# bruAristimunha/Synthetic-Sleep-EEG-Signal-Generation-using-Latent-Diffusion-Models

Measured on AMD Instinct MI355X. Metric: EEG windows/sec (LDM train step), higher is better.
Workload: dtype bf16; 1 GPU; LDM train step on raw (B,1,3072) windows: frozen AutoencoderKL[32,32,64] encode+sample x scale, add_noise, config_ldm.yaml UNet (30.5M params, latent_channels=1) fwd+bwd, epsilon MSE, Adam lr 1e-4 [BASELINE configs[2]/[3]: per-GPU batch 256 = global 2048 / 8]; per_gpu_batch=256, global_batch=256, latent_len=768, parallelism=dp1

## Files before the change

### synthetic-sleep-eeg-signal-generation-using-latent-diffusion-models_amd/csrc/conv_ws.hip

```cpp
#include <stdlib.h>

#include "common.h"
#include "internal.h"

namespace {
constexpr int WS_ROWS = 64;
constexpr int WS_BUF_ROWS = 68;
constexpr int WS_ROW_BYTES = 256;
constexpr int WS_ABUF = WS_BUF_ROWS * WS_ROW_BYTES;
constexpr int WS_OUT = WS_ROWS * WS_ROW_BYTES;
constexpr int WS_RING = 3;
constexpr int WS_LDS = WS_RING * WS_ABUF + WS_OUT;

struct WsArgs {
  const bf16_t* x; long ldx;
  const bf16_t* w; long sWt, sWn, sWk; int tflip;
  const float* bias; const float* rowvec; long ld_rowvec;
  const bf16_t* resid; long ldr;
  bf16_t* y; long ldy;
  int M, L, N, ntiles, tiles_per_block;
  const void* zero_page;
  float* col_parts;
};

typedef unsigned u32x2 __attribute__((ext_vector_type(2)));

__device__ __forceinline__ void ws_barrier() {
  asm volatile("s_waitcnt lgkmcnt(0)" ::: "memory");
  __builtin_amdgcn_s_barrier();
  asm volatile("" ::: "memory");
}

__device__ __forceinline__ void ws_dma16(const void* g, unsigned lds_off) {
  asm volatile("s_mov_b32 m0, %0\n\ts_nop 0\n\tglobal_load_lds_dwordx4 %1, off" ::"s"(lds_off), "v"(g) : "memory", "m0");
}
__device__ __forceinline__ u32x2 ws_load8(const void* g) {
  u32x2 r;
  asm volatile("global_load_dwordx2 %0, %1, off" : "=v"(r) : "v"(g) : "memory");
  return r;
}

__device__ __forceinline__ float ws_row16_sum(float v) {
  v += __builtin_bit_cast(float, __builtin_amdgcn_update_dpp(0, __builtin_bit_cast(int, v), 0xB1, 0xF, 0xF, true));
  v += __builtin_bit_cast(float, __builtin_amdgcn_update_dpp(0, __builtin_bit_cast(int, v), 0x4E, 0xF, 0xF, true));
  v += __builtin_bit_cast(float, __builtin_amdgcn_update_dpp(0, __builtin_bit_cast(int, v), 0x141, 0xF, 0xF, true));
  v += __builtin_bit_cast(float, __builtin_amdgcn_update_dpp(0, __builtin_bit_cast(int, v), 0x140, 0xF, 0xF, true));
  return v;
}
__device__ __forceinline__ void ws_col_stats(float (&cs)[2][4], float (&cq)[2][4], float* __restrict__ row, int n0, int lm, int q) {
#pragma unroll
  for (int cf = 0; cf < 2; cf++)
#pragma unroll
    for (int r = 0; r < 4; r++) {
      const float a = ws_row16_sum(cs[cf][r]), b = ws_row16_sum(cq[cf][r]);
      if (lm == 0) *(float2*)(row + 2 * (n0 + cf * 16 + q * 4 + r)) = make_float2(a, b);
    }
}

template <bool TR, typename T16 = bf16_t, bool ST = false>
__global__ __launch_bounds__(256, 2) void conv3_ws_kernel(const WsArgs p) {
  extern __shared__ __attribute__((aligned(1024))) char smem[];
  const int tid = threadIdx.x, wave = tid >> 6, lane = tid & 63, lm = lane & 15, q = lane >> 4;
  const int n0 = blockIdx.y * 128 + wave * 32;
  const int t_begin = blockIdx.x * p.tiles_per_block;
  int t_end = t_begin + p.tiles_per_block; if (t_end > p.ntiles) t_end = p.ntiles;
  if (t_begin >= t_end) return;
  const unsigned lds_base = (unsigned)(size_t)(__attribute__((address_space(3))) char*)smem;
  const int wave_u = __builtin_amdgcn_readfirstlane(wave);

  auto issue_dma = [&](int t) {
    const int buf = (t - t_begin) % WS_RING;
    const long row0 = (long)t * WS_ROWS;
    const bool has_left = (row0 % p.L) != 0, has_right = ((row0 + WS_ROWS) % p.L) != 0;
    for (int i = wave_u; i < WS_BUF_ROWS / 4; i += 4) {
      const int j = 4 * i + q, c = lm ^ (j & 15);
      const bool ok = (j >= 1 && j <= WS_ROWS) || (j == 0 && has_left) || (j == WS_ROWS + 1 && has_right);
      const char* src = ok ? (const char*)(p.x + (row0 - 1 + j) * p.ldx) + c * 16 : (const char*)p.zero_page;
      ws_dma16(src, __builtin_amdgcn_readfirstlane(lds_base + buf * WS_ABUF + i * 1024));
    }
  };
  issue_dma(t_begin);
  if (t_begin + 1 < t_end) issue_dma(t_begin + 1);

  uint4 wf[3][4][2];
#pragma unroll
  for (int t = 0; t < 3; t++) {
    const bf16_t* wt = p.w + (long)(p.tflip ? 2 - t : t) * p.sWt;
#pragma unroll
    for (int kk = 0; kk < 4; kk++)
#pragma unroll
      for (int cf = 0; cf < 2; cf++) {
        const bf16_t* wp = wt + (long)(n0 + cf * 16 + lm) * p.sWn + (long)(kk * 32 + q * 8) * p.sWk;
        if constexpr (!TR) wf[t][kk][cf] = *(const uint4*)wp;
        else {
          unsigned e[8];
#pragma unroll
          for (int i = 0; i < 8; i++) e[i] = wp[(long)i * p.sWk];
          wf[t][kk][cf] = make_uint4(e[0] | (e[1] << 16), e[2] | (e[3] << 16), e[4] | (e[5] << 16), e[6] | (e[7] << 16));
        }
      }
  }
  float4 bv[2], ev[2];
#pragma unroll
  for (int cf = 0; cf < 2; cf++) bv[cf] = p.bias ? *(const float4*)(p.bias + n0 + cf * 16 + q * 4) : make_float4(0.f, 0.f, 0.f, 0.f);
  int ev_sample = -1;
  __builtin_amdgcn_s_waitcnt(0x0F70);

  char* sOut = smem + WS_RING * WS_ABUF;
  auto store_tile = [&](int t) {
    const long row0 = (long)t * WS_ROWS;
#pragma unroll
    for (int i = 0; i < 4; i++) {
      const int c = tid + 256 * i, row = c >> 4, ch = c & 15;
      const uint4 v = *(const uint4*)(sOut + row * WS_ROW_BYTES + ((ch ^ (row & 15)) * 16));
      *(uint4*)(p.y + (row0 + row) * p.ldy + blockIdx.y * 128 + ch * 8) = v;
    }
  };

  float cs[2][4], cq[2][4];
#pragma unroll
  for (int cf = 0; cf < 2; cf++)
#pragma unroll
    for (int r = 0; r < 4; r++) { cs[cf][r] = 0.f; cq[cf][r] = 0.f; }
  for (int t = t_begin; t < t_end; t++) {
    const int buf = (t - t_begin) % WS_RING;
    const long row0 = (long)t * WS_ROWS;
    if (t + 1 < t_end) asm volatile("s_waitcnt vmcnt(4)" ::: "memory"); else asm volatile("s_waitcnt vmcnt(0)" ::: "memory");
    ws_barrier();
    if (t > t_begin) store_tile(t - 1);
    const int sample = (int)(row0 / p.L);
    if (sample != ev_sample) {
      ev_sample = sample;
#pragma unroll
      for (int cf = 0; cf < 2; cf++) {
        ev[cf] = bv[cf];
        if (p.rowvec) {
          const float4 e = *(const float4*)(p.rowvec + (long)sample * p.ld_rowvec + n0 + cf * 16 + q * 4);
          ev[cf].x += e.x; ev[cf].y += e.y; ev[cf].z += e.z; ev[cf].w += e.w;
        }
      }
    }
    u32x2 rr[4][2];
    if (p.resid) {
#pragma unroll
      for (int rf = 0; rf < 4; rf++)
#pragma unroll
        for (int cf = 0; cf < 2; cf++) rr[rf][cf] = ws_load8(p.resid + (row0 + rf * 16 + lm) * p.ldr + n0 + cf * 16 + q * 4);
    }
    const bool more = t + 2 < t_end;
    if (more) issue_dma(t + 2);

    const char* sA = smem + buf * WS_ABUF;
    f32x4 acc[4][2];
#pragma unroll
    for (int rf = 0; rf < 4; rf++)
#pragma unroll
      for (int cf = 0; cf < 2; cf++) acc[rf][cf] = (f32x4){0.f, 0.f, 0.f, 0.f};
#pragma unroll
    for (int rf = 0; rf < 4; rf++)
#pragma unroll
      for (int tp = 0; tp < 3; tp++) {
        const int j = rf * 16 + lm + tp;
#pragma unroll
        for (int kk = 0; kk < 4; kk++) {
          const uint4 xf = *(const uint4*)(sA + j * WS_ROW_BYTES + (((kk * 4 + q) ^ (j & 15)) * 16));
#pragma unroll
          for (int cf = 0; cf < 2; cf++)
            if constexpr (Is16<T16>::f16) acc[rf][cf] = __builtin_amdgcn_mfma_f32_16x16x32_f16(__builtin_bit_cast(f16x8, wf[tp][kk][cf]), __builtin_bit_cast(f16x8, xf), acc[rf][cf], 0, 0, 0);
            else acc[rf][cf] = __builtin_amdgcn_mfma_f32_16x16x32_bf16(__builtin_bit_cast(bf16x8, wf[tp][kk][cf]), __builtin_bit_cast(bf16x8, xf), acc[rf][cf], 0, 0, 0);
        }
      }
    if (p.resid) {
      if (!more) asm volatile("s_waitcnt vmcnt(0)" ::: "memory");
      asm volatile("s_waitcnt vmcnt(4)" : "+v"(rr[0][0]), "+v"(rr[0][1]), "+v"(rr[1][0]), "+v"(rr[1][1]), "+v"(rr[2][0]), "+v"(rr[2][1]), "+v"(rr[3][0]), "+v"(rr[3][1]) :: "memory");
    }
    ws_barrier();
#pragma unroll
    for (int rf = 0; rf < 4; rf++)
#pragma unroll
      for (int cf = 0; cf < 2; cf++) {
        float v0 = acc[rf][cf][0] + ev[cf].x, v1 = acc[rf][cf][1] + ev[cf].y, v2 = acc[rf][cf][2] + ev[cf].z, v3 = acc[rf][cf][3] + ev[cf].w;
        if (p.resid) {
          v0 += w16_lo<T16>(rr[rf][cf].x); v1 += w16_hi<T16>(rr[rf][cf].x);
          v2 += w16_lo<T16>(rr[rf][cf].y); v3 += w16_hi<T16>(rr[rf][cf].y);
        }
        if constexpr (ST) {
          cs[cf][0] += v0; cs[cf][1] += v1; cs[cf][2] += v2; cs[cf][3] += v3;
          cq[cf][0] = fmaf(v0, v0, cq[cf][0]); cq[cf][1] = fmaf(v1, v1, cq[cf][1]); cq[cf][2] = fmaf(v2, v2, cq[cf][2]); cq[cf][3] = fmaf(v3, v3, cq[cf][3]);
        }
        const int row = rf * 16 + lm, ch = wave * 4 + cf * 2 + (q >> 1);
        *(uint2*)(sOut + row * WS_ROW_BYTES + ((ch ^ (row & 15)) * 16) + (q & 1) * 8) = make_uint2(pack16x2<T16>(v0, v1), pack16x2<T16>(v2, v3));
      }
  }
  ws_barrier();
  store_tile(t_end - 1);
  if constexpr (ST) ws_col_stats(cs, cq, p.col_parts + (size_t)blockIdx.x * 2 * p.N, n0, lm, q);
}

constexpr int W2_ROWS = 32, W2_BUF_ROWS = 36, W2_ROW_BYTES = 512;
constexpr int W2_ABUF = W2_BUF_ROWS * W2_ROW_BYTES;
constexpr int W2_OUT = W2_ROWS * 256;
constexpr int W2_LDS = WS_RING * W2_ABUF + W2_OUT;

struct Ws2Args {
  const bf16_t* x; long ldx;
  const bf16_t* w;
  const float* bias;
  bf16_t* y; long ldy;
  int M, L, ntiles, tiles_per_block;
  const void* zero_page;
  float* col_parts;
};

template <int MODE> struct W2Map;
template <> struct W2Map<0> { static constexpr int SLOTS = 12; static __device__ __forceinline__ void at(int s, int& tp, int& kk) { if (s < 4) { tp = 0; kk = 4 + s; } else { tp = 1; kk = s - 4; } } };
template <> struct W2Map<1> { static constexpr int SLOTS = 8;  static __device__ __forceinline__ void at(int s, int& tp, int& kk) { tp = 1; kk = s; } };
template <> struct W2Map<2> { static constexpr int SLOTS = 16; static __device__ __forceinline__ void at(int s, int& tp, int& kk) { tp = 1 + (s >> 3); kk = s & 7; } };

template <int MODE, typename T16, bool ST = false>
__device__ __forceinline__ void ws2_body(const Ws2Args& p, char* smem) {
  using Map = W2Map<MODE>;
  const int tid = threadIdx.x, wave = tid >> 6, lane = tid & 63, lm = lane & 15, q = lane >> 4;
  const int nb0 = blockIdx.y * 128, n0 = nb0 + wave * 32;
  const int t_begin = blockIdx.x * p.tiles_per_block;
  int t_end = t_begin + p.tiles_per_block; if (t_end > p.ntiles) t_end = p.ntiles;
  if (t_begin >= t_end) return;
  const unsigned lds_base = (unsigned)(size_t)(__attribute__((address_space(3))) char*)smem;
  const int wave_u = __builtin_amdgcn_readfirstlane(wave);
  auto issue_dma = [&](int t) {
    const int buf = (t - t_begin) % WS_RING;
    const long row0 = (long)t * W2_ROWS;
    const bool has_left = (row0 % p.L) != 0, has_right = ((row0 + W2_ROWS) % p.L) != 0;
    for (int i = wave_u; i < W2_BUF_ROWS / 2; i += 4) {
      const int j = 2 * i + (lane >> 5), c = (lane & 31) ^ (j & 15);
      const bool ok = (j >= 1 && j <= W2_ROWS) || (j == 0 && has_left) || (j == W2_ROWS + 1 && has_right);
      const char* src = ok ? (const char*)(p.x + (row0 - 1 + j) * p.ldx) + c * 16 : (const char*)p.zero_page;
      ws_dma16(src, __builtin_amdgcn_readfirstlane(lds_base + buf * W2_ABUF + i * 1024));
    }
  };
  issue_dma(t_begin);
  if (t_begin + 1 < t_end) issue_dma(t_begin + 1);

  uint4 wf[Map::SLOTS][2];
#pragma unroll
  for (int s_ = 0; s_ < Map::SLOTS; s_++) {
    int tp, kk; Map::at(s_, tp, kk);
#pragma unroll
    for (int cf = 0; cf < 2; cf++) {
      const int n = n0 + cf * 16 + lm, k0 = kk * 32 + q * 8;
      if constexpr (MODE == 0) {
        const int tap = k0 < 128 ? 1 : (tp == 0 ? 0 : 2), ci = k0 & 127;
        wf[s_][cf] = *(const uint4*)(p.w + ((long)tap * 256 + n) * 128 + ci);
      } else {
        const int tap = MODE == 1 ? 1 : (tp == 1 ? 2 : 0), ci = n & 127;
        const bf16_t* wp = p.w + ((long)tap * 256 + k0) * 128 + ci;
        unsigned e[8];
#pragma unroll
        for (int i = 0; i < 8; i++) e[i] = wp[(long)i * 128];
        wf[s_][cf] = make_uint4(e[0] | (e[1] << 16), e[2] | (e[3] << 16), e[4] | (e[5] << 16), e[6] | (e[7] << 16));
      }
    }
  }
  float4 bv[2];
#pragma unroll
  for (int cf = 0; cf < 2; cf++) bv[cf] = (MODE == 0 && p.bias) ? *(const float4*)(p.bias + n0 + cf * 16 + q * 4) : make_float4(0.f, 0.f, 0.f, 0.f);
  __builtin_amdgcn_s_waitcnt(0x0F70);

  char* sOut = smem + WS_RING * W2_ABUF;
  auto store_tile = [&](int t) {
    const long row0 = (long)t * W2_ROWS;
#pragma unroll
    for (int i = 0; i < 2; i++) {
      const int c = tid + 256 * i, row = c >> 4, ch = c & 15;
      const uint4 v = *(const uint4*)(sOut + row * 256 + ((ch ^ (row & 15)) * 16));
      *(uint4*)(p.y + (row0 + row) * p.ldy + nb0 + ch * 8) = v;
    }
  };
  float cs[2][4], cq[2][4];
#pragma unroll
  for (int cf = 0; cf < 2; cf++)
#pragma unroll
    for (int r = 0; r < 4; r++) { cs[cf][r] = 0.f; cq[cf][r] = 0.f; }
  for (int t = t_begin; t < t_end; t++) {
    const int buf = (t - t_begin) % WS_RING;
    if (t + 1 < t_end) asm volatile("s_waitcnt vmcnt(4)" ::: "memory"); else asm volatile("s_waitcnt vmcnt(0)" ::: "memory");
    ws_barrier();
    if (t > t_begin) store_tile(t - 1);
    if (t + 2 < t_end) issue_dma(t + 2);
    const char* sA = smem + buf * W2_ABUF;
    f32x4 acc[2][2];
#pragma unroll
    for (int rf = 0; rf < 2; rf++)
#pragma unroll
      for (int cf = 0; cf < 2; cf++) acc[rf][cf] = (f32x4){0.f, 0.f, 0.f, 0.f};
#pragma unroll
    for (int rf = 0; rf < 2; rf++)
#pragma unroll
      for (int s_ = 0; s_ < Map::SLOTS; s_++) {
        int tp, kk; Map::at(s_, tp, kk);
        const int j = rf * 16 + lm + tp;
        const uint4 xf = *(const uint4*)(sA + j * W2_ROW_BYTES + (((kk * 4 + q) ^ (j & 15)) * 16));
#pragma unroll
        for (int cf = 0; cf < 2; cf++)
          if constexpr (Is16<T16>::f16) acc[rf][cf] = __builtin_amdgcn_mfma_f32_16x16x32_f16(__builtin_bit_cast(f16x8, wf[s_][cf]), __builtin_bit_cast(f16x8, xf), acc[rf][cf], 0, 0, 0);
          else acc[rf][cf] = __builtin_amdgcn_mfma_f32_16x16x32_bf16(__builtin_bit_cast(bf16x8, wf[s_][cf]), __builtin_bit_cast(bf16x8, xf), acc[rf][cf], 0, 0, 0);
      }
    ws_barrier();
#pragma unroll
    for (int rf = 0; rf < 2; rf++)
#pragma unroll
      for (int cf = 0; cf < 2; cf++) {
        const float v0 = acc[rf][cf][0] + bv[cf].x, v1 = acc[rf][cf][1] + bv[cf].y, v2 = acc[rf][cf][2] + bv[cf].z, v3 = acc[rf][cf][3] + bv[cf].w;
        if constexpr (ST) {
          cs[cf][0] += v0; cs[cf][1] += v1; cs[cf][2] += v2; cs[cf][3] += v3;
          cq[cf][0] = fmaf(v0, v0, cq[cf][0]); cq[cf][1] = fmaf(v1, v1, cq[cf][1]); cq[cf][2] = fmaf(v2, v2, cq[cf][2]); cq[cf][3] = fmaf(v3, v3, cq[cf][3]);
        }
        const int row = rf * 16 + lm, ch = wave * 4 + cf * 2 + (q >> 1);
        *(uint2*)(sOut + row * 256 + ((ch ^ (row & 15)) * 16) + (q & 1) * 8) = make_uint2(pack16x2<T16>(v0, v1), pack16x2<T16>(v2, v3));
      }
  }
  ws_barrier();
  store_tile(t_end - 1);
  if constexpr (ST) ws_col_stats(cs, cq, p.col_parts + (size_t)blockIdx.x * 2 * 256, n0, lm, q);
}

template <bool DGRAD, typename T16 = bf16_t, bool ST = false>
__global__ __launch_bounds__(256, 2) void conv3_ws2_kernel(const Ws2Args p) {
  extern __shared__ __attribute__((aligned(1024))) char smem[];
  if constexpr (!DGRAD) ws2_body<0, T16, ST>(p, smem);
  else { if (blockIdx.y == 0) ws2_body<1, T16>(p, smem); else ws2_body<2, T16>(p, smem); }
}
}

int conv_ws_try(eegldm_ctx* ctx, int dtype, const void* x, long ldx, const void* w, int Cin, int Cout, int transposed, const float* bias,
                const float* rowvec, long ld_rowvec, const void* resid, long ldr, void* y, long ldy, int B, int L, float* col_parts, int* col_nparts) {
  if (col_nparts) *col_nparts = 0;
  EEG_ENV_VAR(bool, off, getenv("EEGLDM_NO_CONV_WS") != nullptr);
  const int Kred = transposed ? Cout : Cin, N = transposed ? Cin : Cout;
  const long M = (long)B * L;
  if (off || (dtype != EEGLDM_BF16 && dtype != EEGLDM_F16) || Kred != 128 || N % 128 != 0 || L % WS_ROWS != 0 || M >= (1L << 31)) return 0;
  if (ldx % 8 != 0 || ldy % 8 != 0 || (resid && ldr % 4 != 0) || (rowvec && ld_rowvec % 4 != 0)) return 0;
  if (((size_t)x | (size_t)y | (size_t)w) % 16 != 0 || (resid && (size_t)resid % 8 != 0)) return 0;
  constexpr long min_rows = 16384;
  if (M < min_rows) return 0;
  WsArgs a = {};
  a.x = (const bf16_t*)x; a.ldx = ldx; a.w = (const bf16_t*)w;
  if (!transposed) { a.sWt = (long)Cout * Cin; a.sWn = Cin; a.sWk = 1; a.tflip = 0; }
  else { a.sWt = (long)Cout * Cin; a.sWn = 1; a.sWk = Cin; a.tflip = 1; }
  a.bias = bias; a.rowvec = rowvec; a.ld_rowvec = ld_rowvec; a.resid = (const bf16_t*)resid; a.ldr = ldr;
  a.y = (bf16_t*)y; a.ldy = ldy; a.M = (int)M; a.L = L; a.N = N; a.ntiles = (int)(M / WS_ROWS); a.zero_page = ctx->zero_page;
  constexpr int bpc = 2;
  const int ny = N / 128;
  long nbx = (long)ctx->num_cu * bpc / ny; if (nbx < 1) nbx = 1; if (nbx > a.ntiles) nbx = a.ntiles;
  a.tiles_per_block = (int)((a.ntiles + nbx - 1) / nbx);
  nbx = (a.ntiles + a.tiles_per_block - 1) / a.tiles_per_block;
  static DevOnce attr_once;
  if (attr_once.need(ctx->device)) {
    HIP_TRY(hipFuncSetAttribute((const void*)conv3_ws_kernel<false, bf16_t, true>, hipFuncAttributeMaxDynamicSharedMemorySize, WS_LDS));
    HIP_TRY(hipFuncSetAttribute((const void*)conv3_ws_kernel<false, f16_t, true>, hipFuncAttributeMaxDynamicSharedMemorySize, WS_LDS));
    HIP_TRY(hipFuncSetAttribute((const void*)conv3_ws_kernel<false>, hipFuncAttributeMaxDynamicSharedMemorySize, WS_LDS));
    HIP_TRY(hipFuncSetAttribute((const void*)conv3_ws_kernel<true>, hipFuncAttributeMaxDynamicSharedMemorySize, WS_LDS));
    HIP_TRY(hipFuncSetAttribute((const void*)conv3_ws_kernel<false, f16_t>, hipFuncAttributeMaxDynamicSharedMemorySize, WS_LDS));
    HIP_TRY(hipFuncSetAttribute((const void*)conv3_ws_kernel<true, f16_t>, hipFuncAttributeMaxDynamicSharedMemorySize, WS_LDS));
  }
  ProfRec rec; const bool prof = ctx->prof_on;
  if (prof) {
    rec.cls = transposed ? PROF_CONV_DGRAD : PROF_CONV_FWD; rec.flops = 2.0 * (double)M * N * Kred * 3.0;
    rec.M = (int)M; rec.N = N; rec.K = Kred; rec.taps = 3; rec.splitk = 1; rec.kern = "conv_ws";
    HIP_TRY(hipEventCreate(&rec.a)); HIP_TRY(hipEventCreate(&rec.b));
    HIP_TRY(hipEventRecord(rec.a, ctx->stream));
  }
  const bool st = col_parts && col_nparts && !transposed && (size_t)nbx * 2 * N * sizeof(float) <= (16u << 20);
  if (st) {
    a.col_parts = col_parts; *col_nparts = (int)nbx;
    if (dtype == EEGLDM_F16) hipLaunchKernelGGL((conv3_ws_kernel<false, f16_t, true>), dim3((unsigned)nbx, ny), dim3(256), WS_LDS, ctx->stream, a);
    else hipLaunchKernelGGL((conv3_ws_kernel<false, bf16_t, true>), dim3((unsigned)nbx, ny), dim3(256), WS_LDS, ctx->stream, a);
  } else if (dtype == EEGLDM_F16) {
    if (transposed) hipLaunchKernelGGL((conv3_ws_kernel<true, f16_t>), dim3((unsigned)nbx, ny), dim3(256), WS_LDS, ctx->stream, a);
    else hipLaunchKernelGGL((conv3_ws_kernel<false, f16_t>), dim3((unsigned)nbx, ny), dim3(256), WS_LDS, ctx->stream, a);
  } else if (transposed) hipLaunchKernelGGL(conv3_ws_kernel<true>, dim3((unsigned)nbx, ny), dim3(256), WS_LDS, ctx->stream, a);
  else hipLaunchKernelGGL(conv3_ws_kernel<false>, dim3((unsigned)nbx, ny), dim3(256), WS_LDS, ctx->stream, a);
  LAUNCH_CHECK();
  if (prof) { HIP_TRY(hipEventRecord(rec.b, ctx->stream)); ctx->prof.push_back(rec); }
  return 1;
}

int conv_ws2_try(eegldm_ctx* ctx, int dtype, int dgrad, const void* x, const void* w, const float* bias, void* y, int B, int Lo, float* col_parts, int* col_nparts) {
  if (col_nparts) *col_nparts = 0;
  EEG_ENV_VAR(bool, off, getenv("EEGLDM_NO_CONV_WS") != nullptr);
  const long M = (long)B * Lo;
  if (off || (dtype != EEGLDM_BF16 && dtype != EEGLDM_F16) || Lo % W2_ROWS != 0 || M >= (1L << 31) || M < 8192) return 0;
  if (((size_t)x | (size_t)y | (size_t)w) % 16 != 0) return 0;
  Ws2Args a = {};
  a.x = (const bf16_t*)x; a.ldx = 256; a.w = (const bf16_t*)w; a.bias = dgrad ? nullptr : bias; a.y = (bf16_t*)y; a.ldy = 256;
  a.M = (int)M; a.L = Lo; a.ntiles = (int)(M / W2_ROWS); a.zero_page = ctx->zero_page;
  long nbx = (long)ctx->num_cu * 2 / 2; if (nbx < 1) nbx = 1; if (nbx > a.ntiles) nbx = a.ntiles;
  a.tiles_per_block = (int)((a.ntiles + nbx - 1) / nbx);
  nbx = (a.ntiles + a.tiles_per_block - 1) / a.tiles_per_block;
  static DevOnce attr_once;
  if (attr_once.need(ctx->device)) {
    HIP_TRY(hipFuncSetAttribute((const void*)conv3_ws2_kernel<false, bf16_t, true>, hipFuncAttributeMaxDynamicSharedMemorySize, W2_LDS));
    HIP_TRY(hipFuncSetAttribute((const void*)conv3_ws2_kernel<false, f16_t, true>, hipFuncAttributeMaxDynamicSharedMemorySize, W2_LDS));
    HIP_TRY(hipFuncSetAttribute((const void*)conv3_ws2_kernel<false>, hipFuncAttributeMaxDynamicSharedMemorySize, W2_LDS));
    HIP_TRY(hipFuncSetAttribute((const void*)conv3_ws2_kernel<true>, hipFuncAttributeMaxDynamicSharedMemorySize, W2_LDS));
    HIP_TRY(hipFuncSetAttribute((const void*)conv3_ws2_kernel<false, f16_t>, hipFuncAttributeMaxDynamicSharedMemorySize, W2_LDS));
    HIP_TRY(hipFuncSetAttribute((const void*)conv3_ws2_kernel<true, f16_t>, hipFuncAttributeMaxDynamicSharedMemorySize, W2_LDS));
  }
  ProfRec rec; const bool prof = ctx->prof_on;
  if (prof) {
    rec.cls = dgrad ? PROF_CONV_DGRAD : PROF_CONV_FWD; rec.flops = 2.0 * (double)M * 256 * 128 * 3.0;
    rec.M = (int)M; rec.N = 256; rec.K = 128; rec.taps = 3; rec.splitk = 1; rec.kern = "conv_ws2";
    HIP_TRY(hipEventCreate(&rec.a)); HIP_TRY(hipEventCreate(&rec.b)); HIP_TRY(hipEventRecord(rec.a, ctx->stream));
  }
  const dim3 grid((unsigned)nbx, 2);
  const bool st = col_parts && col_nparts && !dgrad && (size_t)nbx * 2 * 256 * sizeof(float) <= (16u << 20);
  if (st) {
    a.col_parts = col_parts; *col_nparts = (int)nbx;
    if (dtype == EEGLDM_F16) hipLaunchKernelGGL((conv3_ws2_kernel<false, f16_t, true>), grid, dim3(256), W2_LDS, ctx->stream, a);
    else hipLaunchKernelGGL((conv3_ws2_kernel<false, bf16_t, true>), grid, dim3(256), W2_LDS, ctx->stream, a);
  } else if (dtype == EEGLDM_F16) {
    if (dgrad) hipLaunchKernelGGL((conv3_ws2_kernel<true, f16_t>), grid, dim3(256), W2_LDS, ctx->stream, a);
    else hipLaunchKernelGGL((conv3_ws2_kernel<false, f16_t>), grid, dim3(256), W2_LDS, ctx->stream, a);
  } else if (dgrad) hipLaunchKernelGGL(conv3_ws2_kernel<true>, grid, dim3(256), W2_LDS, ctx->stream, a);
  else hipLaunchKernelGGL(conv3_ws2_kernel<false>, grid, dim3(256), W2_LDS, ctx->stream, a);
  LAUNCH_CHECK();
  if (prof) { HIP_TRY(hipEventRecord(rec.b, ctx->stream)); ctx->prof.push_back(rec); }
  return 1;
}
```

Baseline: 14280 windows/s.

## Store conv_ws outputs directly via permlane16 swaps instead of LDS staging

Removes the LDS output staging buffer and its extra barrier and store pass. Each lane now rearranges its MFMA results with permlane16_swap so it can write 16-byte rows straight to global memory. Residual loads become 16-byte loads laid out to match. The residual branch becomes a template parameter, the vmcnt waits are generalized to a configurable prefetch depth, and LDS now fits under 64KB so the dynamic-LDS attribute calls are dropped. The cost is more complex wait-count logic and a risk of uncoalesced or wrongly ordered vmcnt accounting.

```diff
diff --git a/synthetic-sleep-eeg-signal-generation-using-latent-diffusion-models_amd/csrc/conv_ws.hip b/synthetic-sleep-eeg-signal-generation-using-latent-diffusion-models_amd/csrc/conv_ws.hip
--- a/synthetic-sleep-eeg-signal-generation-using-latent-diffusion-models_amd/csrc/conv_ws.hip
+++ b/synthetic-sleep-eeg-signal-generation-using-latent-diffusion-models_amd/csrc/conv_ws.hip
@@ -1,16 +1,25 @@
 #include <stdlib.h>
+
+#include <type_traits>
 
 #include "common.h"
 #include "internal.h"
+
+#ifndef EEG_WS_DBG
+#define EEG_WS_DBG 0
+#endif
+#define WS_DBG(b) ((EEG_WS_DBG & (b)) != 0)
 
 namespace {
 constexpr int WS_ROWS = 64;
 constexpr int WS_BUF_ROWS = 68;
 constexpr int WS_ROW_BYTES = 256;
 constexpr int WS_ABUF = WS_BUF_ROWS * WS_ROW_BYTES;
-constexpr int WS_OUT = WS_ROWS * WS_ROW_BYTES;
 constexpr int WS_RING = 3;
-constexpr int WS_LDS = WS_RING * WS_ABUF + WS_OUT;
+constexpr int WS1_RING = 3;
+constexpr int WS1_AHEAD = WS1_RING - 1;
+constexpr int WS_LDS = WS1_RING * WS_ABUF;
+static_assert(WS_LDS <= 64 * 1024 && 8 * WS1_AHEAD + 8 <= 63, "no dynamic-LDS attribute needed; vmcnt holds 63");
 
 struct WsArgs {
   const bf16_t* x; long ldx;
@@ -23,7 +32,8 @@
   float* col_parts;
 };
 
-typedef unsigned u32x2 __attribute__((ext_vector_type(2)));
+typedef unsigned u32x4 __attribute__((ext_vector_type(4)));
+template <typename T> struct WsType { using type = T; };
 
 __device__ __forceinline__ void ws_barrier() {
   asm volatile("s_waitcnt lgkmcnt(0)" ::: "memory");
@@ -34,9 +44,9 @@
 __device__ __forceinline__ void ws_dma16(const void* g, unsigned lds_off) {
   asm volatile("s_mov_b32 m0, %0\n\ts_nop 0\n\tglobal_load_lds_dwordx4 %1, off" ::"s"(lds_off), "v"(g) : "memory", "m0");
 }
-__device__ __forceinline__ u32x2 ws_load8(const void* g) {
-  u32x2 r;
-  asm volatile("global_load_dwordx2 %0, %1, off" : "=v"(r) : "v"(g) : "memory");
+__device__ __forceinline__ u32x4 ws_load16(const void* g) {
+  u32x4 r;
+  asm volatile("global_load_dwordx4 %0, %1, off" : "=v"(r) : "v"(g) : "memory");
   return r;
 }
 
@@ -57,9 +67,12 @@
     }
 }
 
-template <bool TR, typename T16 = bf16_t, bool ST = false>
+template <int N> __device__ __forceinline__ void ws_wait_vm() { asm volatile("s_waitcnt vmcnt(%0)" ::"n"(N) : "memory"); }
+
+template <bool TR, typename T16 = bf16_t, bool ST = false, bool RES = false>
 __global__ __launch_bounds__(256, 2) void conv3_ws_kernel(const WsArgs p) {
   extern __shared__ __attribute__((aligned(1024))) char smem[];
+  static_assert(WS1_AHEAD == 2 || WS1_AHEAD == 3, "the top-of-iteration wait enumerates nd = 0 .. AHEAD - 1");
   const int tid = threadIdx.x, wave = tid >> 6, lane = tid & 63, lm = lane & 15, q = lane >> 4;
   const int n0 = blockIdx.y * 128 + wave * 32;
   const int t_begin = blockIdx.x * p.tiles_per_block;
@@ -69,7 +82,7 @@
   const int wave_u = __builtin_amdgcn_readfirstlane(wave);
 
   auto issue_dma = [&](int t) {
-    const int buf = (t - t_begin) % WS_RING;
+    const int buf = (t - t_begin) % WS1_RING;
     const long row0 = (long)t * WS_ROWS;
     const bool has_left = (row0 % p.L) != 0, has_right = ((row0 + WS_ROWS) % p.L) != 0;
     for (int i = wave_u; i < WS_BUF_ROWS / 4; i += 4) {
@@ -79,8 +92,9 @@
       ws_dma16(src, __builtin_amdgcn_readfirstlane(lds_base + buf * WS_ABUF + i * 1024));
     }
   };
-  issue_dma(t_begin);
-  if (t_begin + 1 < t_end) issue_dma(t_begin + 1);
+#pragma unroll
+  for (int a = 0; a < WS1_AHEAD; a++)
+    if (t_begin + a < t_end) issue_dma(t_begin + a);
 
   uint4 wf[3][4][2];
 #pragma unroll
@@ -91,7 +105,8 @@
 #pragma unroll
       for (int cf = 0; cf < 2; cf++) {
         const bf16_t* wp = wt + (long)(n0 + cf * 16 + lm) * p.sWn + (long)(kk * 32 + q * 8) * p.sWk;
-        if constexpr (!TR) wf[t][kk][cf] = *(const uint4*)wp;
+        if constexpr (WS_DBG(32)) wf[t][kk][cf] = make_uint4(0x3c003c00u + lane, 0x3c003c00u + t, 0x3c003c00u + kk, 0x3c003c00u + cf + tid);
+        else if constexpr (!TR) wf[t][kk][cf] = *(const uint4*)wp;
         else {
           unsigned e[8];
 #pragma unroll
@@ -106,16 +121,7 @@
   int ev_sample = -1;
   __builtin_amdgcn_s_waitcnt(0x0F70);
 
-  char* sOut = smem + WS_RING * WS_ABUF;
-  auto store_tile = [&](int t) {
-    const long row0 = (long)t * WS_ROWS;
-#pragma unroll
-    for (int i = 0; i < 4; i++) {
-      const int c = tid + 256 * i, row = c >> 4, ch = c & 15;
-      const uint4 v = *(const uint4*)(sOut + row * WS_ROW_BYTES + ((ch ^ (row & 15)) * 16));
-      *(uint4*)(p.y + (row0 + row) * p.ldy + blockIdx.y * 128 + ch * 8) = v;
-    }
-  };
+  bf16_t* const yp = p.y + (long)lm * p.ldy + n0 + (q & 1) * 16 + (q >> 1) * 8;
 
   float cs[2][4], cq[2][4];
 #pragma unroll
@@ -123,11 +129,13 @@
 #pragma unroll
     for (int r = 0; r < 4; r++) { cs[cf][r] = 0.f; cq[cf][r] = 0.f; }
   for (int t = t_begin; t < t_end; t++) {
-    const int buf = (t - t_begin) % WS_RING;
+    const int buf = (t - t_begin) % WS1_RING;
     const long row0 = (long)t * WS_ROWS;
-    if (t + 1 < t_end) asm volatile("s_waitcnt vmcnt(4)" ::: "memory"); else asm volatile("s_waitcnt vmcnt(0)" ::: "memory");
+    {
+      int nd = t_end - 1 - t; if (nd > WS1_AHEAD - 1) nd = WS1_AHEAD - 1; if (WS_DBG(1)) nd = 0;
+      if (nd == 0) ws_wait_vm<4 * WS1_AHEAD>(); else if (nd == 1) ws_wait_vm<4 * WS1_AHEAD + 4>(); else ws_wait_vm<4 * WS1_AHEAD + 8>();
+    }
     ws_barrier();
-    if (t > t_begin) store_tile(t - 1);
     const int sample = (int)(row0 / p.L);
     if (sample != ev_sample) {
       ev_sample = sample;
@@ -140,15 +148,14 @@
         }
       }
     }
-    u32x2 rr[4][2];
-    if (p.resid) {
-#pragma unroll
-      for (int rf = 0; rf < 4; rf++)
-#pragma unroll
-        for (int cf = 0; cf < 2; cf++) rr[rf][cf] = ws_load8(p.resid + (row0 + rf * 16 + lm) * p.ldr + n0 + cf * 16 + q * 4);
-    }
-    const bool more = t + 2 < t_end;
-    if (more) issue_dma(t + 2);
+    u32x4 rr[4];
+    constexpr bool has_res = RES && !WS_DBG(8);
+    if (has_res) {
+#pragma unroll
+      for (int rf = 0; rf < 4; rf++) rr[rf] = ws_load16(p.resid + (row0 + rf * 16 + lm) * p.ldr + n0 + (q & 1) * 16 + (q >> 1) * 8);
+    }
+    const bool more = t + WS1_AHEAD < t_end && !WS_DBG(1);
+    if (more) issue_dma(t + WS1_AHEAD);
 
     const char* sA = smem + buf * WS_ABUF;
     f32x4 acc[4][2];
@@ -156,6 +163,7 @@
     for (int rf = 0; rf < 4; rf++)
 #pragma unroll
       for (int cf = 0; cf < 2; cf++) acc[rf][cf] = (f32x4){0.f, 0.f, 0.f, 0.f};
+    if (!WS_DBG(4))
 #pragma unroll
     for (int rf = 0; rf < 4; rf++)
 #pragma unroll
@@ -170,30 +178,39 @@
             else acc[rf][cf] = __builtin_amdgcn_mfma_f32_16x16x32_bf16(__builtin_bit_cast(bf16x8, wf[tp][kk][cf]), __builtin_bit_cast(bf16x8, xf), acc[rf][cf], 0, 0, 0);
         }
       }
-    if (p.resid) {
+    if (has_res) {
       if (!more) asm volatile("s_waitcnt vmcnt(0)" ::: "memory");
-      asm volatile("s_waitcnt vmcnt(4)" : "+v"(rr[0][0]), "+v"(rr[0][1]), "+v"(rr[1][0]), "+v"(rr[1][1]), "+v"(rr[2][0]), "+v"(rr[2][1]), "+v"(rr[3][0]), "+v"(rr[3][1]) :: "memory");
-    }
-    ws_barrier();
-#pragma unroll
-    for (int rf = 0; rf < 4; rf++)
+      else if (wave_u != 0) asm volatile("s_waitcnt vmcnt(4)" ::: "memory");
+      asm volatile("s_waitcnt vmcnt(5)" : "+v"(rr[0]), "+v"(rr[1]), "+v"(rr[2]), "+v"(rr[3]) :: "memory");
+    }
+    bf16_t* const yt = yp + row0 * p.ldy;
+#pragma unroll
+    for (int rf = 0; rf < 4; rf++) {
+      unsigned pk[2][2], rv[2][2];
+      if constexpr (has_res) {
+        const auto r0 = __builtin_amdgcn_permlane16_swap(rr[rf].x, rr[rf].z, false, false);
+        const auto r1 = __builtin_amdgcn_permlane16_swap(rr[rf].y, rr[rf].w, false, false);
+        rv[0][0] = r0[0]; rv[0][1] = r1[0]; rv[1][0] = r0[1]; rv[1][1] = r1[1];
+      }
 #pragma unroll
       for (int cf = 0; cf < 2; cf++) {
         float v0 = acc[rf][cf][0] + ev[cf].x, v1 = acc[rf][cf][1] + ev[cf].y, v2 = acc[rf][cf][2] + ev[cf].z, v3 = acc[rf][cf][3] + ev[cf].w;
-        if (p.resid) {
-          v0 += w16_lo<T16>(rr[rf][cf].x); v1 += w16_hi<T16>(rr[rf][cf].x);
-          v2 += w16_lo<T16>(rr[rf][cf].y); v3 += w16_hi<T16>(rr[rf][cf].y);
+        if constexpr (has_res) {
+          v0 += w16_lo<T16>(rv[cf][0]); v1 += w16_hi<T16>(rv[cf][0]);
+          v2 += w16_lo<T16>(rv[cf][1]); v3 += w16_hi<T16>(rv[cf][1]);
         }
         if constexpr (ST) {
           cs[cf][0] += v0; cs[cf][1] += v1; cs[cf][2] += v2; cs[cf][3] += v3;
           cq[cf][0] = fmaf(v0, v0, cq[cf][0]); cq[cf][1] = fmaf(v1, v1, cq[cf][1]); cq[cf][2] = fmaf(v2, v2, cq[cf][2]); cq[cf][3] = fmaf(v3, v3, cq[cf][3]);
         }
-        const int row = rf * 16 + lm, ch = wave * 4 + cf * 2 + (q >> 1);
-        *(uint2*)(sOut + row * WS_ROW_BYTES + ((ch ^ (row & 15)) * 16) + (q & 1) * 8) = make_uint2(pack16x2<T16>(v0, v1), pack16x2<T16>(v2, v3));
-      }
-  }
-  ws_barrier();
-  store_tile(t_end - 1);
+        pk[cf][0] = pack16x2<T16>(v0, v1); pk[cf][1] = pack16x2<T16>(v2, v3);
+      }
+      const auto s0 = __builtin_amdgcn_permlane16_swap(pk[0][0], pk[1][0], false, false);
+      const auto s1 = __builtin_amdgcn_permlane16_swap(pk[0][1], pk[1][1], false, false);
+      uint4 o; o.x = s0[0]; o.y = s1[0]; o.z = s0[1]; o.w = s1[1];
+      if (!WS_DBG(2) || o.x == 0x12345u) *(uint4*)(yt + (long)rf * 16 * p.ldy) = o;
+    }
+  }
   if constexpr (ST) ws_col_stats(cs, cq, p.col_parts + (size_t)blockIdx.x * 2 * p.N, n0, lm, q);
 }
 
@@ -354,15 +371,6 @@
   long nbx = (long)ctx->num_cu * bpc / ny; if (nbx < 1) nbx = 1; if (nbx > a.ntiles) nbx = a.ntiles;
   a.tiles_per_block = (int)((a.ntiles + nbx - 1) / nbx);
   nbx = (a.ntiles + a.tiles_per_block - 1) / a.tiles_per_block;
-  static DevOnce attr_once;
-  if (attr_once.need(ctx->device)) {
-    HIP_TRY(hipFuncSetAttribute((const void*)conv3_ws_kernel<false, bf16_t, true>, hipFuncAttributeMaxDynamicSharedMemorySize, WS_LDS));
-    HIP_TRY(hipFuncSetAttribute((const void*)conv3_ws_kernel<false, f16_t, true>, hipFuncAttributeMaxDynamicSharedMemorySize, WS_LDS));
-    HIP_TRY(hipFuncSetAttribute((const void*)conv3_ws_kernel<false>, hipFuncAttributeMaxDynamicSharedMemorySize, WS_LDS));
-    HIP_TRY(hipFuncSetAttribute((const void*)conv3_ws_kernel<true>, hipFuncAttributeMaxDynamicSharedMemorySize, WS_LDS));
-    HIP_TRY(hipFuncSetAttribute((const void*)conv3_ws_kernel<false, f16_t>, hipFuncAttributeMaxDynamicSharedMemorySize, WS_LDS));
-    HIP_TRY(hipFuncSetAttribute((const void*)conv3_ws_kernel<true, f16_t>, hipFuncAttributeMaxDynamicSharedMemorySize, WS_LDS));
-  }
   ProfRec rec; const bool prof = ctx->prof_on;
   if (prof) {
     rec.cls = transposed ? PROF_CONV_DGRAD : PROF_CONV_FWD; rec.flops = 2.0 * (double)M * N * Kred * 3.0;
@@ -371,15 +379,20 @@
     HIP_TRY(hipEventRecord(rec.a, ctx->stream));
   }
   const bool st = col_parts && col_nparts && !transposed && (size_t)nbx * 2 * N * sizeof(float) <= (16u << 20);
-  if (st) {
-    a.col_parts = col_parts; *col_nparts = (int)nbx;
-    if (dtype == EEGLDM_F16) hipLaunchKernelGGL((conv3_ws_kernel<false, f16_t, true>), dim3((unsigned)nbx, ny), dim3(256), WS_LDS, ctx->stream, a);
-    else hipLaunchKernelGGL((conv3_ws_kernel<false, bf16_t, true>), dim3((unsigned)nbx, ny), dim3(256), WS_LDS, ctx->stream, a);
-  } else if (dtype == EEGLDM_F16) {
-    if (transposed) hipLaunchKernelGGL((conv3_ws_kernel<true, f16_t>), dim3((unsigned)nbx, ny), dim3(256), WS_LDS, ctx->stream, a);
-    else hipLaunchKernelGGL((conv3_ws_kernel<false, f16_t>), dim3((unsigned)nbx, ny), dim3(256), WS_LDS, ctx->stream, a);
-  } else if (transposed) hipLaunchKernelGGL(conv3_ws_kernel<true>, dim3((unsigned)nbx, ny), dim3(256), WS_LDS, ctx->stream, a);
-  else hipLaunchKernelGGL(conv3_ws_kernel<false>, dim3((unsigned)nbx, ny), dim3(256), WS_LDS, ctx->stream, a);
+  if (st) { a.col_parts = col_parts; *col_nparts = (int)nbx; }
+  const dim3 grid((unsigned)nbx, ny);
+  hipStream_t stream = ctx->stream;
+  auto launch = [&](auto kern) { hipLaunchKernelGGL(kern, grid, dim3(256), WS_LDS, stream, a); };
+  auto pick_res = [&](auto tr, auto t16, auto stc) {
+    constexpr bool TR = decltype(tr)::value, STC = decltype(stc)::value; using T = typename decltype(t16)::type;
+    if (resid) launch(conv3_ws_kernel<TR, T, STC, true>); else launch(conv3_ws_kernel<TR, T, STC, false>);
+  };
+  auto pick_t = [&](auto tr, auto stc) {
+    if (dtype == EEGLDM_F16) pick_res(tr, WsType<f16_t>{}, stc); else pick_res(tr, WsType<bf16_t>{}, stc);
+  };
+  if (st) pick_t(std::false_type{}, std::true_type{});
+  else if (transposed) pick_t(std::true_type{}, std::false_type{});
+  else pick_t(std::false_type{}, std::false_type{});
   LAUNCH_CHECK();
   if (prof) { HIP_TRY(hipEventRecord(rec.b, ctx->stream)); ctx->prof.push_back(rec); }
   return 1;
```

New measurement: 14310 windows/s (median of 6 runs). Within noise of the previous version (+0.2%).
